# jonnylaw/bayesian_dlms

Measured on AMD Instinct MI355X. Metric: Kalman filter+smooth series*timesteps/sec, higher is better.
Workload: dtype f64

## Files before the change

### bayesian_dlms_amd/csrc/dlm_engine.hip

```cpp
#include "../../include/dlm_engine.h"
#include <cstdlib>
#include "dlm_internal.h"
#include "dlm_draws.h"

#include <rccl/rccl.h>

#include <cstdio>
#include <cstring>
#include <map>
#include <mutex>
#include <set>
#include <string>
#include <vector>

using dlm::KArgs;

namespace dlm {
namespace {
struct LdsEntry {
  size_t granted = 0;
  long long whole = -1;
};
std::mutex lds_mutex;
std::map<std::pair<const void*, int>, LdsEntry> lds_book;
size_t limit_locked(int dev) {
  LdsEntry& lim = lds_book[{nullptr, dev}];
  if (!lim.granted) {
    int v = 0;
    if (hipDeviceGetAttribute(&v, hipDeviceAttributeMaxSharedMemoryPerBlock, dev) != hipSuccess) { (void)hipGetLastError(); v = 0; }
    lim.granted = v > 0 ? (size_t)v : 0;
  }
  return lim.granted;
}
hipError_t opt_in_locked(const void* fn, int dev, size_t bytes) {
  if (bytes > limit_locked(dev)) return hipErrorInvalidValue;
  LdsEntry& en = lds_book[{fn, dev}];
  if (bytes <= en.granted) return hipSuccess;
  const hipError_t err = hipFuncSetAttribute(fn, hipFuncAttributeMaxDynamicSharedMemorySize, (int)bytes);
  if (err == hipSuccess) en.granted = bytes;
  return err;
}
}
size_t lds_limit() {
  int dev = 0;
  if (hipGetDevice(&dev) != hipSuccess) { (void)hipGetLastError(); return 0; }
  std::lock_guard<std::mutex> lock(lds_mutex);
  return limit_locked(dev);
}
hipError_t lds_opt_in(const void* fn, size_t bytes) {
  int dev = 0;
  const hipError_t err = hipGetDevice(&dev);
  if (err != hipSuccess) return err;
  std::lock_guard<std::mutex> lock(lds_mutex);
  return opt_in_locked(fn, dev, bytes);
}
size_t whole_cu_lds(const void* fn) {
  int dev = 0;
  if (hipGetDevice(&dev) != hipSuccess) { (void)hipGetLastError(); return 0; }
  std::lock_guard<std::mutex> lock(lds_mutex);
  LdsEntry& en = lds_book[{fn, dev}];
  if (en.whole < 0) {
    en.whole = 0;
    hipFuncAttributes at;
    const size_t whole = limit_locked(dev);
    if (hipFuncGetAttributes(&at, fn) != hipSuccess) (void)hipGetLastError();
    else if (at.sharedSizeBytes < whole) {
      if (opt_in_locked(fn, dev, whole - at.sharedSizeBytes) == hipSuccess) en.whole = (long long)(whole - at.sharedSizeBytes);
      else (void)hipGetLastError();
    }
  }
  return (size_t)en.whole;
}
}

struct Workspace {
  void* p = nullptr;
  size_t bytes = 0;
  Workspace* next;
  explicit Workspace(Workspace*& list) : next(list) { list = this; }
};
template <class T>
struct Ws : Workspace {
  using Workspace::Workspace;
  operator T*() const { return (T*)p; }
};

struct dlm_engine {
  int device = 0;
  hipStream_t own_stream = nullptr;
  hipStream_t stream = nullptr;
  std::string err;
  const char* variant = "none";
  hipEvent_t ev[3] = {nullptr, nullptr, nullptr};
  bool timed = false;
  Workspace* workspaces = nullptr;
  Ws<void> arena{workspaces};
  Ws<dlm::SparseT> sp_dev{workspaces};
  Ws<dlm::SparseBig> spb_dev{workspaces};
  Ws<double> fws{workspaces}, side{workspaces}, xplus{workspaces}, ystar{workspaces}, covws{workspaces};
  Ws<unsigned char> route{workspaces}, plainbuf{workspaces};
  Ws<void> sampws{workspaces};
  Ws<double> zws{workspaces};
  Ws<void> rtsws{workspaces};
  dlm::SparseF* spf_dev = nullptr;
  int sparse_k = 0;
  ncclComm_t comm = nullptr;
  bool has_comm = false;
  std::set<void*> buffers;
  hipEvent_t order_ev = nullptr;
  struct Analysis {
    bool valid = false;
    int d = 0, p = 0, n_g = 0, branch = 0;
    long long f_stride = 0;
    unsigned generic = 0;
    int sparse_k = 0, spb_k = 0, spf_k = 0;
    bool have_spb = false, have_spf = false;
    std::vector<double> g_host, f_host;
  } an;
  bool an_touched = true;
  bool rts_last = false;
  hipStream_t rng_stream = nullptr;
  hipEvent_t rng_ev = nullptr;
  hipStream_t cov_stream = nullptr;
  hipEvent_t cov_ev[2] = {nullptr, nullptr};
// ... 324 lines not shown
  HIP_TRY(e, hipMemcpyAsync(e->sp_dev, tabs.data(), tabs.size() * sizeof(dlm::SparseT), hipMemcpyHostToDevice, e->stream));
  HIP_TRY(e, hipStreamSynchronize(e->stream));
  e->sparse_k = K;
  return DLM_OK;
}

int mark(dlm_engine* e, int i) {
  HIP_TRY(e, hipEventRecord(e->ev[i], e->stream));
  if (i == 2) e->timed = true;
  return DLM_OK;
}

int ensure_side(dlm_engine* e, size_t N, size_t T) { return ensure(e, e->side, sizeof(double) * 3 * N * (T + 1)); }

int ensure_xplus(dlm_engine* e, const KArgs& k) { return ensure(e, e->xplus, sizeof(double) * (size_t)k.N * ((size_t)k.T + 1) * (size_t)k.d); }

int ensure_ystar(dlm_engine* e, const KArgs& k) {
  return ensure(e, e->ystar, sizeof(double) * (size_t)k.N * (size_t)k.T * (size_t)k.p + (((size_t)k.N * (size_t)(k.T + 1) + 15) & ~(size_t)15));
}

int packed_path(dlm_engine* e, KArgs& k) {
  k.flags |= DLM_OPT_NO_LANE;
  if (!(fast_shape_ok(k) && e->sparse_k > 0) || (k.flags & DLM_OPT_SMOOTHER_COMPAT_Q1))
    return fail(e, DLM_ERR_UNSUPPORTED, "DLM_OPT_PACKED_SYM needs the structured d <= 15, p = 1 path (time-invariant F, <= 4 nonzeros per row and column of G) without DLM_OPT_FORCE_GENERIC / DLM_OPT_SMOOTHER_COMPAT_Q1; use dense records otherwise");
  return DLM_OK;
}

bool use_shared_cov(const dlm_engine* e, const KArgs& k) {
  return fast_shape_ok(k) && e->sparse_k > 0 && !dlm::lane_supported(k) && dlm::shared_cov_eligible(k);
}
size_t route_pad(size_t N) { return (N + 63) & ~(size_t)63; }
int ensure_route(dlm_engine* e, size_t N) { return ensure(e, e->route, route_pad(N) + N * sizeof(int)); }
int* leave_of(dlm_engine* e, size_t N) { return (int*)(e->route + route_pad(N)); }
int mark_plain(dlm_engine* e, KArgs& k) {
  k.plain = nullptr;
  if (!(fast_shape_ok(k) && e->sparse_k > 0) || use_lane(k) || !k.y || k.g_index || k.dt || k.f_stride || k.v_tstride || k.w_tstride ||
      (k.flags & DLM_OPT_NO_STEADY)) return DLM_OK;
  { const int rc = ensure(e, e->plainbuf, (size_t)k.N); if (rc) return rc; }
  HIP_TRY(e, dlm::launch_sparse16_count_gaps(k, e->plainbuf, e->stream));
  k.plain = e->plainbuf;
  return DLM_OK;
}
int ensure_cov_stream(dlm_engine* e) {
  if (!e->cov_stream) {
    int lo = 0, hi = 0;
    HIP_TRY(e, hipDeviceGetStreamPriorityRange(&lo, &hi));
    HIP_TRY(e, hipStreamCreateWithPriority(&e->cov_stream, hipStreamNonBlocking, hi));
    for (auto& ev : e->cov_ev) HIP_TRY(e, hipEventCreateWithFlags(&ev, hipEventDisableTiming));
    HIP_TRY(e, hipEventCreateWithFlags(&e->cov_ev2, hipEventDisableTiming));
    HIP_TRY(e, hipEventCreateWithFlags(&e->rts_ev, hipEventDisableTiming));
  }
  return DLM_OK;
}
int start_sampler_normals(dlm_engine* e, const KArgs& k, dlm::SampTabs& tb, bool big, hipEvent_t gate);
int start_sampler_tables(dlm_engine* e, const KArgs& k, dlm::SampTabs& tb, bool big, const double* crec = nullptr, int crec_stride = 0, bool defer_normals = false) {
  int rc = ensure(e, e->sampws, big ? dlm::wave48_sampler_shared_ws_bytes(k) : dlm::sampler_shared_ws_bytes(k));
  if (rc || (rc = ensure_route(e, (size_t)k.N)) || (rc = ensure_cov_stream(e))) return rc;
  if (big) dlm::wave48_sampler_shared_carve(e->sampws, k, tb); else dlm::sampler_shared_carve(e->sampws, k, tb);
  if ((rc = aux_fork(e, e->cov_stream, e->cov_busy, e->cov_ev[0]))) return rc;
  tb.zstride = 0; tb.mc4 = nullptr; tb.marked = 0;
  if (big) HIP_TRY(e, dlm::launch_wave48_sampler_shared_tables(k, tb, e->cov_stream, e->cov_ev2));
  else if (crec) HIP_TRY(e, dlm::launch_sampler_shared_tables_from(k, e->sparse_k, e->sp_dev, tb, crec, crec_stride, e->cov_stream));
  else HIP_TRY(e, dlm::launch_sampler_shared_tables(k, e->sparse_k, e->sp_dev, tb, e->cov_stream));
  tb.z4 = nullptr;
  if (defer_normals) return DLM_OK;
  return start_sampler_normals(e, k, tb, big, e->cov_ev[0]);
}
int start_sampler_normals(dlm_engine* e, const KArgs& k, dlm::SampTabs& tb, bool big, hipEvent_t gate) {
  if (!k.z) {
    int rc = ensure(e, e->zws, big ? dlm::wave48_sampler_shared_normals_bytes(k) : dlm::sampler_shared_normals_bytes(k));
    if (rc) return rc;
    if (!e->rng_stream) {
      HIP_TRY(e, hipStreamCreateWithFlags(&e->rng_stream, hipStreamNonBlocking));
      HIP_TRY(e, hipEventCreateWithFlags(&e->rng_ev, hipEventDisableTiming));
    }
    if ((rc = aux_fork(e, e->rng_stream, e->rng_busy, gate, false))) return rc;
    if (big) HIP_TRY(e, dlm::launch_wave48_sampler_shared_normals(k, e->zws, e->rng_stream));
    else HIP_TRY(e, dlm::launch_sampler_shared_normals(k, e->zws, e->rng_stream));
    tb.z4 = e->zws;
  }
  return DLM_OK;
}
int start_rts_tables(dlm_engine* e, const KArgs& k, dlm::RtsTabs& tb) {
  bool fresh = false;
  int rc = ensure(e, e->rtsws, dlm::rts_shared_ws_bytes(k), &fresh);
  if (rc) return rc;
  if (fresh) HIP_TRY(e, hipMemsetAsync(e->rtsws, 0, 64, e->stream));
  if ((rc = ensure(e, e->covws, sizeof(double) * dlm::covtabs_doubles(k.d, k.T)))) return rc;
  if ((rc = ensure_route(e, (size_t)k.N)) || (rc = ensure_cov_stream(e))) return rc;
  dlm::RtsKeep keep{};
  dlm::rts_shared_carve(e->rtsws, k, tb, keep);
  dlm::CovTabs ctb{};
  dlm::covtabs_carve(e->covws, k.d, k.T, ctb);
  const bool no_reuse = (k.flags & DLM_OPT_NO_TABLE_REUSE) != 0;
  const int* gate = keep.ctl + dlm::RTS_CTL_GATE;
  e->rts_last = true;
  HIP_TRY(e, dlm::launch_rts_shared_mark(k, e->route, tb, e->stream));
  HIP_TRY(e, dlm::launch_rts_key_check(k, e->sparse_k, e->sp_dev, keep, no_reuse, e->stream));
  HIP_TRY(e, dlm::launch_rts_shared_cov(k, e->sparse_k, e->sp_dev, tb, ctb, gate, e->stream));
  if ((rc = aux_fork(e, e->cov_stream, e->cov_busy, e->cov_ev[0]))) return rc;
  HIP_TRY(e, dlm::launch_rts_shared_tables(k, e->sparse_k, e->sp_dev, tb, gate, e->cov_stream));
  HIP_TRY(e, dlm::launch_rts_key_commit(k, e->sparse_k, e->sp_dev, keep, no_reuse, e->cov_stream));
  HIP_TRY(e, hipEventRecord(e->rts_ev, e->cov_stream));
  HIP_TRY(e, dlm::launch_rts_broadcast(k, e->route, tb, e->cov_stream));
  return DLM_OK;
}
int ensure_shared(dlm_engine* e, const KArgs& k, dlm::CovTabs& tb, bool with_backward) {
  int rc = ensure(e, e->covws, sizeof(double) * dlm::covtabs_doubles(k.d, k.T));
  if (rc || (rc = ensure_route(e, (size_t)k.N)) || (rc = ensure_side(e, k.N, k.T)) || (rc = ensure_cov_stream(e))) return rc;
  dlm::covtabs_carve(e->covws, k.d, k.T, tb);
  tb.eq = e->side + 2 * (size_t)k.N * ((size_t)k.T + 1);
  tb.mc = tb.sc = nullptr;
  if (with_backward) {
    const size_t one = 64 * (size_t)((k.N + 3) / 4) * ((size_t)k.T + 1);
    if ((rc = ensure(e, e->xplus, sizeof(double) * one))) return rc;
    tb.mc = e->xplus;
  }
  return DLM_OK;
}
int run_shared_filter(dlm_engine* e, KArgs& k, dlm::CovTabs& tb, bool with_backward) {
  int rc = ensure_shared(e, k, tb, with_backward);
  if (rc) return rc;
  k.route = e->route; k.route_take = 0;
  e->variant = "sparse16";
  HIP_TRY(e, dlm::launch_sparse16_cov_filter(k, e->sparse_k, e->sp_dev, tb, e->stream));
  if (with_backward) {
    if ((rc = aux_fork(e, e->cov_stream, e->cov_busy, e->cov_ev[0]))) return rc;
    HIP_TRY(e, dlm::launch_sparse16_cov_smoother(k, e->sparse_k, e->sp_dev, tb, e->cov_stream));
  }
  HIP_TRY(e, dlm::launch_sparse16_mean_filter(k, e->sparse_k, e->sp_dev, tb, e->stream));
  KArgs kg = k;
  kg.route_take = 1;
  HIP_TRY(e, dlm::launch_sparse16_filter(kg, e->sparse_k, e->sp_dev, with_backward ? e->side : nullptr, nullptr, e->stream));
  return DLM_OK;
}
int run_shared_smoother(dlm_engine* e, KArgs& k, const dlm::CovTabs& tb) {
  { const int rc = join_cov(e); if (rc) return rc; }
  HIP_TRY(e, dlm::launch_sparse16_mean_smoother(k, e->sparse_k, e->sp_dev, tb, e->stream));
  KArgs kg = k;
  kg.route_take = 1;
  HIP_TRY(e, dlm::launch_sparse16_smoother(kg, e->sparse_k, e->sp_dev, e->side, e->stream));
  return DLM_OK;
}

int run_filter(dlm_engine* e, const KArgs& k, bool want_side) {
  if (use_lane(k)) {
    e->variant = "lane";
    HIP_TRY(e, dlm::launch_lane_filter(k, e->stream));
  } else if (use_fast(e, k) && (!k.prior || e->sparse_k)) {
    if (want_side) { int rc = ensure_side(e, k.N, k.T); if (rc) return rc; }
    double* side = want_side ? e->side : nullptr;
    if (e->sparse_k) {
      e->variant = "sparse16";
      HIP_TRY(e, dlm::launch_sparse16_filter(k, e->sparse_k, e->sp_dev, side, nullptr, e->stream));
    } else {
      e->variant = "mfma16";
      HIP_TRY(e, dlm::launch_mfma16_filter(k, side, e->stream));
// ... 954 lines not shown
  if ((rc = mark(e, 2))) return rc;
  return st.finish(opts->flags & DLM_OPT_ASYNC);
}

int dlm_filter_smooth_batch(dlm_engine* e, const dlm_model_desc* model,
                            const dlm_params_desc* params, const double* y,
                            const dlm_options* opts, double* filt, double* smooth,
                            int32_t* status) {
  int rc = check_common(e, model, params, opts);
  if (rc) return rc;
  if (!y || !smooth) return fail(e, DLM_ERR_ARG, "y and smooth are required");
  e->rts_last = false;
  AuxScope aux(e);
  const size_t d = model->d, p = model->p, T = model->T, N = model->N, rec = d + d * d;
  KArgs k{};
  Stager st(e, opts->mem == DLM_MEM_HOST);
  stage_model(st, k, model, params, opts);
  const bool want_packed = (opts->flags & DLM_OPT_PACKED_SYM) != 0;
  const size_t orec = want_packed ? (size_t)dlm_packed_record_doubles((int)d) : rec;
  st.in(&k.y, y, N * T * p);
  st.out(&k.filt, filt, filt ? N * (T + 1) * orec : 0);
  st.out(&k.smooth, smooth, N * (T + 1) * orec);
  st.zeroed_out(&k.status, (int*)status, N);
  if ((rc = st.commit())) return rc;
  if ((rc = analyse_g(e, k, model->G, opts->mem == DLM_MEM_HOST))) return rc;
  if (want_packed && (rc = packed_path(e, k))) return rc;
  bool fused_fast = fast_smoother_ok(e, k) || use_tiled(k);
  if (want_packed) k.packed = 3;
  const bool q1 = (k.flags & DLM_OPT_SMOOTHER_COMPAT_Q1) != 0;
  const bool rts_shared = fast_shape_ok(k) && e->sparse_k > 0 && !use_lane(k) && !k.packed && !(k.flags & DLM_OPT_SHARED_COV) &&
                          (q1 ? !fused_fast : fast_smoother_ok(e, k)) && dlm::rts_shared_eligible(k, !q1) &&
                          ((uintptr_t)k.smooth & 15) == 0;
  if (!filt) {
    k.packed |= (fast_smoother_ok(e, k) && e->sparse_k > 0 && !use_lane(k) && !rts_shared) ? 1 : 0;
    if ((rc = ensure(e, e->fws, (k.packed & 1) ? N * (T + 1) * (size_t)dlm::packed_rec_bytes((int)d) : N * (T + 1) * rec * sizeof(double)))) return rc;
    k.filt = e->fws;
  }
  if ((rc = mark(e, 0))) return rc;
  dlm::RtsTabs rtb{};
  if (rts_shared && (rc = start_rts_tables(e, k, rtb))) return rc;
  if (rts_shared && (k.flags & DLM_OPT_TEST_FAIL_AFTER_TABLES))
    return fail(e, DLM_ERR_UNSUPPORTED, "DLM_OPT_TEST_FAIL_AFTER_TABLES");
  if ((rc = mark_plain(e, k))) return rc;
  if (filt && fast_smoother_ok(e, k) && use_shared_cov(e, k)) {
    dlm::CovTabs tb;
    if ((rc = run_shared_filter(e, k, tb, true))) return rc;
    if ((rc = mark(e, 1))) return rc;
    k.filt_in = k.filt;
    if ((rc = run_shared_smoother(e, k, tb))) return rc;
    if ((rc = mark(e, 2))) return rc;
    return st.finish(opts->flags & DLM_OPT_ASYNC);
  }
  if ((rc = run_filter(e, k, fused_fast))) return rc;
  if (rts_shared) HIP_TRY(e, hipStreamWaitEvent(e->stream, e->rts_ev, 0));
  if ((rc = mark(e, 1))) return rc;
  k.filt_in = k.filt;
  if (rts_shared) {
    k.route = e->route; k.route_take = 0;
    e->variant = "sparse16-rts-shared";
    HIP_TRY(e, dlm::launch_rts_shared_means(k, e->sparse_k, e->sp_dev, rtb, q1, e->stream));
    if (!q1) {
      KArgs kg = k;
      kg.route_take = 1;
      HIP_TRY(e, dlm::launch_sparse16_smoother(kg, e->sparse_k, e->sp_dev, e->side, e->stream));
    }
  } else if ((rc = run_smoother(e, k, fused_fast))) return rc;
  if (rts_shared && (rc = join_cov(e))) return rc;
  if ((rc = mark(e, 2))) return rc;
  return st.finish(opts->flags & DLM_OPT_ASYNC);
}

static int simsmooth_lane(dlm_engine* e, KArgs& k) {
  int rc = ensure_xplus(e, k);
  if (rc) return rc;
  e->variant = "lane-simsmooth";
  HIP_TRY(e, dlm::launch_lane_simsmooth(k, e->xplus, e->stream));
  return (rc = mark(e, 1)) ? rc : mark(e, 2);
}
static int simsmooth_sparse16(dlm_engine* e, KArgs& k) {
  int rc;
  if ((rc = ensure_side(e, k.N, k.T)) || (rc = ensure_xplus(e, k))) return rc;
  e->variant = "sparse16-simsmooth";
  HIP_TRY(e, dlm::launch_sparse16_filter(k, e->sparse_k, e->sp_dev, e->side, e->xplus, e->stream));
  if ((rc = mark(e, 1))) return rc;
  k.filt_in = k.filt;
  HIP_TRY(e, dlm::launch_sparse16_simsmooth(k, e->sparse_k, e->sp_dev, e->side, e->xplus, e->stream));
  return mark(e, 2);
}
static int simsmooth_tiled(dlm_engine* e, KArgs& k) {
  int rc;
  if (k.w_tstride) {
    k.flags |= DLM_OPT_FORCE_WAVE;
    if (!dlm::wave48_simsmooth_supported(k))
      return fail(e, DLM_ERR_UNSUPPORTED, "a W_t stream with DLM_OPT_FFBS_SIMSMOOTH needs a structured G (at most four nonzeros per row and column); the reference-form sampler takes any model");
  }
  if ((rc = ensure_xplus(e, k)) || (rc = ensure_ystar(e, k))) return rc;
  e->variant = dlm::wave48_simsmooth_supported(k) ? "wave-simsmooth" : "tiled-simsmooth";
  HIP_TRY(e, dlm::launch_tiled_simsmooth(k, e->xplus, e->ystar, e->stream));
  return (rc = mark(e, 1)) ? rc : mark(e, 2);
}
static int forward_shared_means(dlm_engine* e, KArgs& k, dlm::SampTabs& stb) {
  int rc;
  dlm::CovTabs ctb;
  if ((rc = ensure_shared(e, k, ctb, true))) return rc;
  k.route = e->route; k.route_take = 0; k.filt = nullptr;
  HIP_TRY(e, dlm::launch_sparse16_cov_filter(k, e->sparse_k, e->sp_dev, ctb, e->stream));
  if ((rc = start_sampler_tables(e, k, stb, false, ctb.ftab, ctb.frow))) return rc;
  if (k.flags & DLM_OPT_TEST_FAIL_AFTER_TABLES) return fail(e, DLM_ERR_UNSUPPORTED, "DLM_OPT_TEST_FAIL_AFTER_TABLES");
  HIP_TRY(e, dlm::launch_sparse16_mean_filter(k, e->sparse_k, e->sp_dev, ctb, e->stream));
  stb.mc4 = ctb.mc;
  KArgs kg = k;
  kg.route_take = 1; kg.filt = e->fws;
  HIP_TRY(e, dlm::launch_sparse16_filter(kg, e->sparse_k, e->sp_dev, nullptr, nullptr, e->stream));
  k.filt_in = e->fws;
  return DLM_OK;
}
static int forward_records(dlm_engine* e, KArgs& k, dlm::SampTabs& stb, bool shared_factors, bool shared_big, bool norec_big) {
  int rc;
  if ((shared_factors || shared_big) && (rc = start_sampler_tables(e, k, stb, shared_big, nullptr, 0, norec_big))) return rc;
  if ((shared_factors || shared_big) && (k.flags & DLM_OPT_TEST_FAIL_AFTER_TABLES))
// ... 244 lines not shown
```

### bayesian_dlms_amd/csrc/dlm_internal.h

```cpp
#pragma once
#include <hip/hip_runtime.h>
#include <stdint.h>
#include <type_traits>
#include "../../include/dlm_engine.h"

namespace dlm {

struct KArgs {
  int d, p, T, N;
  const double* F; long long f_stride;
  const double* G; int n_g; const int* g_index; const double* dt;
  const double* V; long long v_stride;
  const double* W; long long w_stride;
  long long v_tstride, w_tstride;
  const double* m0; long long m0_stride;
  const double* C0; long long c0_stride;
  const double* y;
  const double* z;
  const double* filt_in;
  double* filt;
  double* prior;
  double* fq;
  double* smooth;
  double* theta;
// ... 114 lines not shown
  double* zrec;
  double* zeros;
  unsigned char* need;
  int* status;
  double* z4;
  int zstride;
  const double* mc4;
  int marked;
  double* ktab;
  int* settle;
};
bool sampler_shared_model_ok(const KArgs& a);
bool sampler_shared_eligible(const KArgs& a);
size_t sampler_shared_ws_bytes(const KArgs& a);
void sampler_shared_carve(void* ws, const KArgs& a, SampTabs& tb);
hipError_t launch_sampler_shared_tables(const KArgs& a, int K, const SparseT* tabs_dev, const SampTabs& tb, hipStream_t s);
hipError_t launch_sampler_shared_tables_from(const KArgs& a, int K, const SparseT* tabs_dev, SampTabs tb, const double* crec, int stride, hipStream_t s);
size_t sampler_shared_normals_bytes(const KArgs& a);
hipError_t launch_sampler_shared_normals(const KArgs& a, double* z4, hipStream_t s);
hipError_t launch_sampler_shared_draw(const KArgs& a, int K, const SparseT* tabs_dev, const SampTabs& tb, hipStream_t s);

struct RtsTabs {
  double* jrows;
  double* srec;
  unsigned char* need;
  int* status;
  const double* crec;
  int crec_stride;
  int* gaps;
  int* skip;
};
constexpr unsigned RTS_KEY_FLAGS = (1u << 0) | (1u << 22);
struct RtsKeySrc {
  int d, T, K;
  unsigned flags;
  const double *F, *V, *W, *C0;
  const SparseT* sp;
};
enum { RTS_CTL_HIT = 10,
       RTS_CTL_GATE = 11,
       RTS_CTL_VALID = 12,
       RTS_CTL_LAST = 13 };
struct RtsKeep { int* ctl; unsigned* key; };
constexpr int RTS_KEY_WORDS = 8 + 2 * (15 + 1 + 2 * 15 * 15) + 2 * (int)(sizeof(SparseT) / 4);
bool rts_shared_eligible(const KArgs& a, bool textbook);
size_t rts_shared_ws_bytes(const KArgs& a);
void rts_shared_carve(void* ws, const KArgs& a, RtsTabs& tb, RtsKeep& keep);
hipError_t launch_rts_key_check(const KArgs& a, int K, const SparseT* tabs_dev, const RtsKeep& keep, bool no_reuse, hipStream_t s);
hipError_t launch_rts_key_commit(const KArgs& a, int K, const SparseT* tabs_dev, const RtsKeep& keep, bool no_reuse, hipStream_t s);
hipError_t launch_rts_shared_cov(const KArgs& a, int K, const SparseT* tabs_dev, RtsTabs& tb, const CovTabs& ctb, const int* gate, hipStream_t s);
hipError_t launch_rts_shared_tables(const KArgs& a, int K, const SparseT* tabs_dev, const RtsTabs& tb, const int* gate, hipStream_t s);
hipError_t launch_rts_shared_mark(const KArgs& a, unsigned char* route, const RtsTabs& tb, hipStream_t s);
hipError_t launch_rts_shared_means(const KArgs& a, int K, const SparseT* tabs_dev, const RtsTabs& tb, bool own_rts, hipStream_t s);
hipError_t launch_rts_broadcast(const KArgs& a, const unsigned char* route, const RtsTabs& tb, hipStream_t s);

bool wave48_sampler_shared_model_ok(const KArgs& a);
bool wave48_sampler_shared_eligible(const KArgs& a);
size_t wave48_sampler_shared_ws_bytes(const KArgs& a);
void wave48_sampler_shared_carve(void* ws, const KArgs& a, SampTabs& tb);
hipError_t launch_wave48_sampler_shared_tables(const KArgs& a, const SampTabs& tb, hipStream_t s, hipEvent_t after_filter = nullptr);
hipError_t launch_wave48_sampler_shared_draw(const KArgs& a, const SampTabs& tb, hipStream_t s);
size_t wave48_ktab_doubles(const KArgs& a);
hipError_t launch_wave48_steady_filter(const KArgs& a, const double* ktab, const int* settle, hipStream_t s);
hipError_t launch_wave48_mark_gaps(const KArgs& a, unsigned char* route, hipStream_t s);
size_t wave48_sampler_shared_normals_bytes(const KArgs& a);
hipError_t launch_wave48_sampler_shared_normals(const KArgs& a, double* z, hipStream_t s);

struct SparseBig { int K; int pad; int idx[48][4]; double val[48][4]; };
int sparse48_analyse(const double* G_host, int d, SparseBig* rows, SparseBig* cols);
struct SparseF { int K; int pad; int cidx[32][4]; double cval[32][4]; int ridx[48][4]; double rval[48][4]; };
int sparsef_analyse(const double* F_host, int d, int p, SparseF* out);
bool tiled_supported(const KArgs& a);
hipError_t launch_tiled_filter(const KArgs& a, double* innov, hipStream_t s);
hipError_t launch_tiled_smoother(const KArgs& a, const double* innov, hipStream_t s);
bool wave48_small_shape(const KArgs& a);
bool wave48_small_ok(const KArgs& a);
bool wave48_filter_supported(const KArgs& a);
hipError_t launch_wave48_filter(const KArgs& a, int K, double* innov, hipStream_t s);
bool wave48_smoother_supported(const KArgs& a);
hipError_t launch_wave48_smoother(const KArgs& a, int K, const double* innov, hipStream_t s);
bool wave48_simsmooth_supported(const KArgs& a);
hipError_t launch_wave48_simsmooth(const KArgs& a, int K, double* xplus, double* ystar, hipStream_t s);
bool wave48_sampler_supported(const KArgs& a);
hipError_t launch_wave48_sampler(const KArgs& a, hipStream_t s);
hipError_t launch_tiled_simsmooth(const KArgs& a, double* xplus, double* ystar, hipStream_t s);

bool svd_supported(const KArgs& a);
size_t svd_filter_lds_bytes(int d, int p);
hipError_t launch_svd_filter(const KArgs& a, double* svd_rec, hipStream_t s);
hipError_t launch_svd_sampler(const KArgs& a, const double* svd_rec, hipStream_t s);
bool svd_shared_eligible(const KArgs& a);
size_t svd_shared_ws_doubles(const KArgs& a);
hipError_t launch_svd_filter_shared(const KArgs& a, double* svd_rec, double* ws, unsigned char* route, hipStream_t s);

bool lane_supported(const KArgs& a);
hipError_t launch_lane_filter(const KArgs& a, hipStream_t s);
hipError_t launch_lane_smoother(const KArgs& a, hipStream_t s);
hipError_t launch_lane_sampler(const KArgs& a, hipStream_t s);
hipError_t launch_lane_simsmooth(const KArgs& a, double* xplus, hipStream_t s);

hipError_t launch_ar1_ffbs(int N, int T, const double* times, const double* y, const double* v, long long v_stride,
                           const double* sv, long long sv_stride, const double* z, unsigned long long seed,
                           unsigned long long series_offset, double* filt, double* theta, int* status, hipStream_t s);

struct DrawStream { unsigned long long seed, series_offset, iteration; };

hipError_t launch_dinvgamma_step(int d, int p, int N, const double* stats, double av, double bv, double aw, double bw,
// ... 255 lines not shown
```

### bayesian_dlms_amd/csrc/dlm_sampler16.hip

```cpp
#include "dlm_internal.h"
#include "dlm_wave.h"
#include "../../include/dlm_engine.h"

namespace dlm {
namespace s16 {

constexpr int IL = 17;
constexpr int IMG = 16 * IL;

__device__ __forceinline__ d4 mm(const d4& x, const d4& y, int rows) {
  d4 acc = {0.0, 0.0, 0.0, 0.0};
#pragma unroll
  for (int r = 0; r < 4; ++r)
    if (4 * r < rows) acc = __builtin_amdgcn_mfma_f64_16x16x4f64(x[r], y[r], acc, 0, 0, 0);
  return acc;
}
__device__ __forceinline__ void to_img(const d4& x, double* img, int g, int c) {
#pragma unroll
  for (int r = 0; r < 4; ++r) img[(4 * r + g) * IL + c] = x[r];
}
__device__ __forceinline__ d4 transposed(const d4& x, double* img, int g, int c) {
  to_img(x, img, g, c);
  wave_sync();
  d4 y;
// ... 982 lines not shown
  if (nd1) lds_dma<NRJ>(rjt, jring_lds + ((T - 1) & 1) * (RJ_ROW * 8), (T - 1) * (RJ_ROW * 8), lane, nj16);
  double sc;
  {
    vm_wait<0>();
    wave_sync();
    const unsigned sslot = sring_lds + (T & 1) * RT_SLOT, mslot = mring_lds + (T & (SF_AHEAD - 1)) * 512;
    double mr = lds_read64<0>(mslot + lane * 8), td = lds_read64<0>(sslot + ptd);
    asm volatile("s_waitcnt lgkmcnt(0)" : "+v"(mr), "+v"(td)::"memory");
    sc = vc ? mr : 0.0;
    vH[lane] = vc ? mr : td;
    wave_sync();
    emit(T, sslot, jring_lds + (T & 1) * (RJ_ROW * 8), mslot, nd2);
  }
  for (int t = T - 1; t >= 0; --t) {
    nd0 = nd1; nd1 = nd2; nd2 = need_of(t - 2);
    if (nd1) vm_wait<4 + NRJ>(); else vm_wait<4>();
    const unsigned sslot = sring_lds + (t & 1) * RT_SLOT, jslot = jring_lds + (t & 1) * (RJ_ROW * 8), mslot = mring_lds + (t & (SF_AHEAD - 1)) * 512;
    double mr = lds_read64<0>(mslot + lane * 8), td = lds_read64<0>(sslot + ptd);
    double mg[K];
#pragma unroll
    for (int s = 0; s < K; ++s) mg[s] = lds_read64<0>(mslot + idx[s]);
    if constexpr (K == 1) asm volatile("s_waitcnt lgkmcnt(0)" : "+v"(mr), "+v"(td), "+v"(mg[0])::"memory");
    else if constexpr (K == 2) asm volatile("s_waitcnt lgkmcnt(0)" : "+v"(mr), "+v"(td), "+v"(mg[0]), "+v"(mg[1])::"memory");
    else if constexpr (K == 3) asm volatile("s_waitcnt lgkmcnt(0)" : "+v"(mr), "+v"(td), "+v"(mg[0]), "+v"(mg[1]), "+v"(mg[2])::"memory");
    else asm volatile("s_waitcnt lgkmcnt(0)" : "+v"(mr), "+v"(td), "+v"(mg[0]), "+v"(mg[1]), "+v"(mg[2]), "+v"(mg[3])::"memory");
    if (nd0) read_J(jslot);
    const double mc = vc ? mr : 0.0;
    double a1 = 0.0;
#pragma unroll
    for (int s = 0; s < K; ++s) a1 = fma(vc ? mg[s] : 0.0, val[s], a1);
    vU[lane] = vc ? sc - a1 : 0.0;
    wave_sync();
    double ch[4] = {0.0, 0.0, 0.0, 0.0};
#pragma unroll
    for (int r = 0; r < 4; ++r)
#pragma unroll
      for (int g = 0; g < 4; ++g) ch[g] = fma(Jc[4 * r + g], vU[16 * j + 4 * r + g], ch[g]);
    const double scol = mc + ((ch[0] + ch[1]) + (ch[2] + ch[3]));
    vH[lane] = vc ? scol : td;
    wave_sync();
    emit(t, sslot, jslot, mslot, nd2);
    sc = vc ? scol : 0.0;
  }
  vm_wait<0>();
  const int stz = tb.status[0];
  const unsigned long long badl = __ballot(!dead && vc && !isfinite(sc));
  if (!dead && c == 0) {
    const int sj = stz | (((badl >> (16 * j)) & 0xffffull) ? DLM_ST_NONFINITE : 0);
    if (a.status && sj) atomicOr(&a.status[n], sj);
  }
}

__global__ __launch_bounds__(256) void k_rts_broadcast(const double* __restrict__ srec, double* smooth, const unsigned char* __restrict__ route,
                                                       const int* __restrict__ skip, int N, int T, int d, int nch) {
  const int lane = threadIdx.x & 63, w = __builtin_amdgcn_readfirstlane((int)(blockIdx.x * 4 + (threadIdx.x >> 6)));
  if (w >= (T + 1) * nch || *skip != 0) return;
  const int t = w % (T + 1), ch = w / (T + 1);
  const int per = (N + nch - 1) / nch, nb = ch * per, ne = nb + per < N ? nb + per : N;
  const int recb = (d + d * d) * 8;
  const bool lines = rts_split_lines(recb), last = t == T;
  const size_t sbytes = (size_t)(T + 1) * recb;
  d2 pc[2];
  int po[2];
#pragma unroll
  for (int k = 0; k < 2; ++k) {
    const int o = 128 + 16 * (64 * k + lane);
    po[k] = o < recb ? o : -1;
    pc[k] = d2{0.0, 0.0};
    if (o < recb) pc[k] = *(const d2*)((const char*)srec + (size_t)t * recb + o);
  }
  unsigned long long routed = 0;
  for (int n = nb; n < ne; ++n) {
    const int i = (n - nb) & 63;
    if (i == 0) routed = __ballot(n + lane < ne && route[n + lane] != 0);
    if ((routed >> i) & 1ull) continue;
    const __amdgpu_buffer_rsrc_t r = mk_rsrc((char*)smooth + (size_t)n * sbytes, sbytes);
    const int ph = (int)(((unsigned long long)smooth + (unsigned long long)n * sbytes + (unsigned long long)t * recb) & 127ull);
#pragma unroll
    for (int k = 0; k < 2; ++k) bst128(r, (po[k] >= 0 && !rts_head_piece(po[k], ph, recb, lines, last)) ? po[k] : OOB, t * recb, pc[k]);
  }
}

}

template <class Tab>
static hipError_t launch_sampler_t(const KArgs& a, int K, const Tab* tabs_dev, hipStream_t s) {
  return pick<1, 2, 3, 4>(K, [&](auto k) { return launch(s16::k_sampler_sp16<k(), Tab>, dim3(a.N), dim3(64), 0, s, a, tabs_dev, SampTabs{}); });
}
hipError_t launch_sparse16_sampler(const KArgs& a, int K, const SparseT* tabs_dev, hipStream_t s) { return launch_sampler_t(a, K, tabs_dev, s); }

template <class Tab>
static hipError_t launch_rts_t(const KArgs& a, int K, const Tab* tabs_dev, hipStream_t s) {
  return pick<1, 2, 3, 4>(K, [&](auto k) { return launch(s16::k_smoother_rts16<k(), Tab>, dim3(a.N), dim3(64), 0, s, a, tabs_dev, RtsTabs{}); });
}
#ifndef DLM_SAMPLER_SHARED_MIN
#define DLM_SAMPLER_SHARED_MIN 1
#endif
bool sampler_shared_model_ok(const KArgs& a) {
  const size_t rec = (size_t)a.d + (size_t)a.d * a.d;
  return a.d <= 15 && a.p == 1 && !a.g_index && !a.dt && !a.f_stride && !a.v_tstride && !a.w_tstride && !a.v_stride && !a.w_stride && !a.c0_stride &&
         !a.packed && a.T >= 1 && a.T <= 400000 && 4 * ((size_t)a.T + 1) * rec * 8 < ((size_t)1 << 31);
}
bool sampler_shared_eligible(const KArgs& a) {
  return sampler_shared_model_ok(a) && !a.cond && (!a.stats || a.y) &&
         !(a.flags & (DLM_OPT_STATS_OUTER | DLM_OPT_FORCE_GENERIC | DLM_OPT_NO_SAMPLER16 | DLM_OPT_SAMPLER_PER_SERIES)) &&
         (a.N >= DLM_SAMPLER_SHARED_MIN || (a.flags & DLM_OPT_NO_SMALL_BATCH));
}
static size_t up64(size_t x) { return (x + 63) & ~(size_t)63; }
size_t sampler_shared_ws_bytes(const KArgs& a) {
  const size_t n1 = (size_t)a.T + 1, rec = (size_t)a.d + (size_t)a.d * a.d;
  return up64(n1 * s16::SF_ROW * 8) + up64(n1 * rec * 8) + up64((size_t)(a.T > 16 ? a.T : 16) * 8) + up64(n1) + 64;
}
void sampler_shared_carve(void* ws, const KArgs& a, SampTabs& tb) {
  const size_t n1 = (size_t)a.T + 1, rec = (size_t)a.d + (size_t)a.d * a.d;
  char* p = (char*)ws;
  tb.rows = (double*)p;  p += up64(n1 * s16::SF_ROW * 8);
  tb.zrec = (double*)p;  p += up64(n1 * rec * 8);
  tb.zeros = (double*)p; p += up64((size_t)(a.T > 16 ? a.T : 16) * 8);
  tb.need = (unsigned char*)p; p += up64(n1);
  tb.status = (int*)p; tb.settle = tb.status + 1;
}
static hipError_t launch_sampler_table_run(const KArgs& kp, int K, const SparseT* tabs_dev, const SampTabs& tb, hipStream_t s) {
  const dim3 grid(s16::sf_stretches(kp.T));
  return pick<1, 2, 3, 4>(K, [&](auto k) { return launch(s16::k_sampler_sp16<k(), SparseT, true>, grid, dim3(64), 0, s, kp, tabs_dev, tb); });
}
hipError_t launch_sampler_shared_tables(const KArgs& a, int K, const SparseT* tabs_dev, const SampTabs& tb, hipStream_t s) {
  hipError_t err = hipMemsetAsync(tb.zeros, 0, (size_t)(a.T > 16 ? a.T : 16) * 8, s);
  if (err != hipSuccess) return err;
  if ((err = hipMemsetAsync(tb.status, 0, sizeof(int), s)) != hipSuccess) return err;
  KArgs kf = table_run_args(a);
  kf.y = tb.zeros; kf.m0 = tb.zeros; kf.filt = tb.zrec; kf.status = tb.status;
  if ((err = launch_sparse16_filter(kf, K, tabs_dev, nullptr, nullptr, s)) != hipSuccess) return err;
// ... 74 lines not shown
  const size_t n1 = (size_t)a.T + 1, rec = (size_t)a.d + (size_t)a.d * a.d;
  return 64 + rts_key_bytes() + up64(n1 * s16::RJ_ROW * 8) + up64(n1 * rec * 8) + up64(n1);
}
void rts_shared_carve(void* ws, const KArgs& a, RtsTabs& tb, RtsKeep& keep) {
  const size_t n1 = (size_t)a.T + 1, rec = (size_t)a.d + (size_t)a.d * a.d;
  char* p = (char*)ws;
  keep.ctl = (int*)p; p += 64;
  keep.key = (unsigned*)p; p += rts_key_bytes();
  tb.jrows = (double*)p; p += up64(n1 * s16::RJ_ROW * 8);
  tb.srec = (double*)p;  p += up64(n1 * rec * 8);
  tb.need = (unsigned char*)p;
  tb.status = keep.ctl; tb.gaps = tb.status + 8; tb.skip = tb.status + 9;
  tb.crec = nullptr; tb.crec_stride = 0;
}
static RtsKeySrc rts_key_of(const KArgs& a, int K, const SparseT* tabs_dev) {
  RtsKeySrc s;
  s.d = a.d; s.T = a.T; s.K = K; s.flags = a.flags & RTS_KEY_FLAGS;
  s.F = a.F; s.V = a.V; s.W = a.W; s.C0 = a.C0; s.sp = tabs_dev;
  return s;
}
hipError_t launch_rts_key_check(const KArgs& a, int K, const SparseT* tabs_dev, const RtsKeep& keep, bool no_reuse, hipStream_t s) {
  if (a.d < 1 || a.d > 15) return hipErrorInvalidValue;
  return launch(s16::k_rts_key_check, dim3(1), dim3(256), 0, s, rts_key_of(a, K, tabs_dev), (const unsigned*)keep.key, keep.ctl, no_reuse ? 1 : 0);
}
hipError_t launch_rts_key_commit(const KArgs& a, int K, const SparseT* tabs_dev, const RtsKeep& keep, bool no_reuse, hipStream_t s) {
  if (a.d < 1 || a.d > 15) return hipErrorInvalidValue;
  return launch(s16::k_rts_key_commit, dim3(1), dim3(256), 0, s, rts_key_of(a, K, tabs_dev), keep.key, keep.ctl, no_reuse ? 1 : 0);
}
hipError_t launch_rts_shared_cov(const KArgs& a, int K, const SparseT* tabs_dev, RtsTabs& tb, const CovTabs& ctb, const int* gate, hipStream_t s) {
  tb.crec = ctb.ftab; tb.crec_stride = ctb.frow;
  CovTabs cs = ctb;
  cs.skip = gate;
  return launch_sparse16_cov_filter(a, K, tabs_dev, cs, s);
}
hipError_t launch_rts_shared_tables(const KArgs& a, int K, const SparseT* tabs_dev, const RtsTabs& tb0, const int* gate, hipStream_t s) {
  RtsTabs tb = tb0;
  tb.skip = const_cast<int*>(gate);
  KArgs kp = table_run_args(a);
  kp.smooth = tb.srec; kp.status = tb.status;
  return pick<1, 2, 3, 4>(K, [&](auto k) {
    const auto kernel = s16::k_smoother_rts16<k(), SparseT, true>;
    return launch(kernel, dim3(1), dim3(64), whole_cu_lds((const void*)kernel), s, kp, tabs_dev, tb);
  });
}
template <int K>
static hipError_t launch_mean_rts(const KArgs& a, const SparseT* sp, const RtsTabs& tb, hipStream_t s) {
  const dim3 grid((a.N + 3) / 4), blk(64);
  constexpr int shape[5][3] = {{2, 1, 1}, {4, 1, 2}, {6, 2, 2}, {8, 2, 2}, {8, 2, 3}};
  const int d = a.d;
  return pick<0, 1, 2, 3, 4>(d <= 7 ? 0 : d <= 10 ? 1 : d <= 13 ? 2 : d == 14 ? 3 : 4, [&](auto c) {
    return launch(s16::k_mean_rts16<K, shape[c()][0], shape[c()][1], shape[c()][2]>, grid, blk, 0, s, a, sp, tb);
  });
}
hipError_t launch_rts_broadcast(const KArgs& a, const unsigned char* route, const RtsTabs& tb, hipStream_t s) {
  if (!route || !a.smooth || a.d < 1 || a.d > 15) return hipErrorInvalidValue;
  const long long rows = (long long)a.T + 1;
  long long nch = (2048 + rows - 1) / rows;
  if (nch > a.N) nch = a.N;
  if (nch < 1) nch = 1;
  return launch(s16::k_rts_broadcast, dim3((unsigned)((rows * nch + 3) / 4)), dim3(256), 0, s, (const double*)tb.srec, a.smooth, route, (const int*)tb.skip, a.N, a.T, a.d, (int)nch);
}
hipError_t launch_rts_shared_mark(const KArgs& a, unsigned char* route, const RtsTabs& tb, hipStream_t s) {
  if (!route || !a.y) return hipErrorInvalidValue;
  hipError_t err = hipMemsetAsync(tb.gaps, 0, 2 * sizeof(int), s);
  if (err != hipSuccess) return err;
  if ((err = launch(s16::k_mark_gaps, dim3((a.N + 3) / 4), dim3(256), 0, s, a.y, a.N, a.T, route, tb.gaps)) != hipSuccess) return err;
  return launch(s16::k_rts_decide, dim3((a.N + 255) / 256), dim3(256), 0, s, route, a.N, (const int*)tb.gaps, tb.skip);
}
hipError_t launch_rts_shared_means(const KArgs& a, int K, const SparseT* tabs_dev, const RtsTabs& tb, bool own_rts, hipStream_t s) {
  if (!a.route || !a.y) return hipErrorInvalidValue;
  hipError_t err;
  KArgs km = a;
  km.route_take = 0;
  err = pick<1, 2, 3, 4>(K, [&](auto k) { return launch_mean_rts<k()>(km, tabs_dev, tb, s); });
  if (err != hipSuccess || !own_rts) return err;
  KArgs kg = a;
  kg.route_take = 1;
  return launch_rts_t(kg, K, tabs_dev, s);
}

hipError_t launch_sparse16_rts(const KArgs& a, int K, const SparseT* tabs_dev, hipStream_t s) { return launch_rts_t(a, K, tabs_dev, s); }
hipError_t launch_small_mv_rts(const KArgs& a, hipStream_t s) { return launch_rts_t(a, a.spb_k, a.spb, s); }
hipError_t launch_small_mv_sampler(const KArgs& a, hipStream_t s) { return launch_sampler_t(a, a.spb_k, a.spb, s); }

}
```

### bayesian_dlms_amd/csrc/dlm_wave.h

```cpp
#pragma once
#include "dlm_internal.h"

namespace dlm {

typedef double d4 __attribute__((ext_vector_type(4)));
typedef double d2 __attribute__((ext_vector_type(2)));
typedef unsigned u2 __attribute__((ext_vector_type(2)));
typedef unsigned u4 __attribute__((ext_vector_type(4)));
typedef int i4 __attribute__((ext_vector_type(4)));

__device__ __forceinline__ void wave_sync() {
  __builtin_amdgcn_fence(__ATOMIC_RELEASE, "wavefront");
  __builtin_amdgcn_wave_barrier();
  __builtin_amdgcn_fence(__ATOMIC_ACQUIRE, "wavefront");
}

template <int CTRL>
__device__ __forceinline__ double dpp_mov(double v) {
  int lo = __double2loint(v), hi = __double2hiint(v);
  lo = __builtin_amdgcn_update_dpp(0, lo, CTRL, 0xf, 0xf, true);
  hi = __builtin_amdgcn_update_dpp(0, hi, CTRL, 0xf, 0xf, true);
  return __hiloint2double(hi, lo);
}
template <int N>
// ... 49 lines not shown
  const u2 l = __builtin_amdgcn_permlane16_swap((unsigned)__double2loint(x), (unsigned)__double2loint(y), false, false);
  const u2 h = __builtin_amdgcn_permlane16_swap((unsigned)__double2hiint(x), (unsigned)__double2hiint(y), false, false);
  lo = __hiloint2double((int)h[0], (int)l[0]);
  hi = __hiloint2double((int)h[1], (int)l[1]);
}
__device__ __forceinline__ double readlane_d(double v, int src) {
  const int lo = __builtin_amdgcn_readlane((int)__double2loint(v), src);
  const int hi = __builtin_amdgcn_readlane((int)__double2hiint(v), src);
  return __hiloint2double(hi, lo);
}
__device__ __forceinline__ double row_pick(double v, int lane, int src) {
  const int a_ = ((lane & 48) + src) << 2;
  const int lo = __builtin_amdgcn_ds_bpermute(a_, __double2loint(v)), hi = __builtin_amdgcn_ds_bpermute(a_, __double2hiint(v));
  return __hiloint2double(hi, lo);
}
__device__ __forceinline__ double row_lane0(double v, int lane) {
  const int a = (lane & 48) << 2;
  const int lo = __builtin_amdgcn_ds_bpermute(a, __double2loint(v)), hi = __builtin_amdgcn_ds_bpermute(a, __double2hiint(v));
  return __hiloint2double(hi, lo);
}

__device__ __forceinline__ double fast_rcp(double x) {
  double r = __builtin_amdgcn_rcp(x);
  r = fma(fma(-x, r, 1.0), r, r);
  r = fma(fma(-x, r, 1.0), r, r);
  return r;
}

__device__ __forceinline__ d4 mmT(const d4& x, const d4& y) {
  d4 acc = {0.0, 0.0, 0.0, 0.0};
  acc = __builtin_amdgcn_mfma_f64_16x16x4f64(x[0], y[0], acc, 0, 0, 0);
  acc = __builtin_amdgcn_mfma_f64_16x16x4f64(x[1], y[1], acc, 0, 0, 0);
  acc = __builtin_amdgcn_mfma_f64_16x16x4f64(x[2], y[2], acc, 0, 0, 0);
  acc = __builtin_amdgcn_mfma_f64_16x16x4f64(x[3], y[3], acc, 0, 0, 0);
  return acc;
}

constexpr int OOB = 0x7ffffff0;
__device__ __forceinline__ __amdgpu_buffer_rsrc_t mk_rsrc(const void* p, size_t bytes) {
  return __builtin_amdgcn_make_buffer_rsrc(const_cast<void*>(p), 0, (int)bytes, 0x00020000);
}
__device__ __forceinline__ double bld(__amdgpu_buffer_rsrc_t r, int voff, int soff) {
  const u2 v = __builtin_amdgcn_raw_buffer_load_b64(r, voff, soff, 0);
  return __hiloint2double((int)v[1], (int)v[0]);
}
__device__ __forceinline__ double bld_glc(__amdgpu_buffer_rsrc_t r, int voff, int soff) {
  const u2 v = __builtin_amdgcn_raw_buffer_load_b64(r, voff, soff, 1);
  return __hiloint2double((int)v[1], (int)v[0]);
}
__device__ __forceinline__ void bst(__amdgpu_buffer_rsrc_t r, int voff, int soff, double x) {
  const u2 v = {(unsigned)__double2loint(x), (unsigned)__double2hiint(x)};
  __builtin_amdgcn_raw_buffer_store_b64(v, r, voff, soff, 0);
}
__device__ __forceinline__ d2 bld128(__amdgpu_buffer_rsrc_t r, int voff, int soff) {
  const u4 v = __builtin_amdgcn_raw_buffer_load_b128(r, voff, soff, 0);
  d2 o = {__hiloint2double((int)v[1], (int)v[0]), __hiloint2double((int)v[3], (int)v[2])};
  return o;
}
template <int AUX = 0>
__device__ __forceinline__ void bst128(__amdgpu_buffer_rsrc_t r, int voff, int soff, double x, double y) {
  const u4 v = {(unsigned)__double2loint(x), (unsigned)__double2hiint(x), (unsigned)__double2loint(y), (unsigned)__double2hiint(y)};
  __builtin_amdgcn_raw_buffer_store_b128(v, r, voff, soff, AUX);
}
template <int AUX = 0>
__device__ __forceinline__ void bst128(__amdgpu_buffer_rsrc_t r, int voff, int soff, d2 x) { bst128<AUX>(r, voff, soff, x[0], x[1]); }

__device__ __forceinline__ i4 rsrc_words(const void* p, unsigned bytes) {
  const unsigned long long a = (unsigned long long)p;
  i4 r = {__builtin_amdgcn_readfirstlane((int)(unsigned)a), __builtin_amdgcn_readfirstlane((int)(unsigned)((a >> 32) & 0xffffu)),
          __builtin_amdgcn_readfirstlane((int)bytes), 0x00020000};
  return r;
}
__device__ __forceinline__ unsigned lds_addr_of(const void* p) {
  return (unsigned)(size_t)(__attribute__((address_space(3))) const char*)p;
}
__device__ __forceinline__ void lds_dma_issue(const i4& rs, unsigned lds_addr, int voff, int soff) {
  asm volatile("s_mov_b32 m0, %0\n\ts_nop 0\n\tbuffer_load_dwordx4 %1, %2, %3 offen lds" ::"s"(lds_addr), "v"(voff), "s"(rs), "s"(soff) : "memory");
}
template <int NR>
__device__ __forceinline__ void lds_dma(const i4& rs, unsigned lds_addr, int soff, int lane, int n16) {
  static_assert(NR >= 1 && NR <= 4, "at most 256 pieces");
  const int voff = lane * 16;
  lds_addr = (unsigned)__builtin_amdgcn_readfirstlane((int)lds_addr);
  soff = __builtin_amdgcn_readfirstlane(soff);
  if (lane < n16) asm volatile("s_mov_b32 m0, %0\n\ts_nop 0\n\tbuffer_load_dwordx4 %1, %2, %3 offen lds" ::"s"(lds_addr), "v"(voff), "s"(rs), "s"(soff) : "memory");
  if constexpr (NR > 1) if (lane + 64 < n16) asm volatile("s_mov_b32 m0, %0\n\ts_nop 0\n\tbuffer_load_dwordx4 %1, %2, %3 offen offset:1024 lds" ::"s"(lds_addr), "v"(voff), "s"(rs), "s"(soff) : "memory");
  if constexpr (NR > 2) if (lane + 128 < n16) asm volatile("s_mov_b32 m0, %0\n\ts_nop 0\n\tbuffer_load_dwordx4 %1, %2, %3 offen offset:2048 lds" ::"s"(lds_addr), "v"(voff), "s"(rs), "s"(soff) : "memory");
  if constexpr (NR > 3) if (lane + 192 < n16) asm volatile("s_mov_b32 m0, %0\n\ts_nop 0\n\tbuffer_load_dwordx4 %1, %2, %3 offen offset:3072 lds" ::"s"(lds_addr), "v"(voff), "s"(rs), "s"(soff) : "memory");
}

template <int OFF>
__device__ __forceinline__ double lds_read64(unsigned addr) {
  double v;
  asm volatile("ds_read_b64 %0, %1 offset:%2" : "=v"(v) : "v"(addr), "n"(OFF) : "memory");
  return v;
}
template <int OFF = 0>
__device__ __forceinline__ d2 lds_read128(unsigned addr) {
  d2 v;
  asm volatile("ds_read_b128 %0, %1 offset:%2" : "=v"(v) : "v"(addr), "n"(OFF) : "memory");
  return v;
}
__device__ __forceinline__ void lds_fence(d4& a) { asm volatile("s_waitcnt lgkmcnt(0)" : "+v"(a)::"memory"); }
__device__ __forceinline__ void lds_fence(d4& a, d4& b) { asm volatile("s_waitcnt lgkmcnt(0)" : "+v"(a), "+v"(b)::"memory"); }
__device__ __forceinline__ void lds_wait(d2& a) { asm volatile("s_waitcnt lgkmcnt(0)" : "+v"(a)::"memory"); }
__device__ __forceinline__ void lds_wait(d2& a, d2& b, d2& c) { asm volatile("s_waitcnt lgkmcnt(0)" : "+v"(a), "+v"(b), "+v"(c)::"memory"); }
// ... 30 lines not shown
```

Baseline: 1.771 billion.

## Make RTS broadcast a CU-sized persistent grid with fixed chunks and pacing

Rewrites the RTS table broadcast kernel as a grid-stride loop over fixed 64-series chunks, with the grid capped at a few blocks per CU. When the table key check hits, the kernel runs alongside the forward filter, so it uses fewer waves in that case. Route bytes and table rows are read through buffer loads, and stores are paced with vm_wait. A compile-time option moves the launch onto the rng stream after the filter, but the default keeps it on the cov stream. The aim is to cut bandwidth contention with the concurrent filter and reduce the cost of oversized launches, at the price of less parallelism in the broadcast.

```diff
diff --git a/bayesian_dlms_amd/csrc/dlm_engine.hip b/bayesian_dlms_amd/csrc/dlm_engine.hip
--- a/bayesian_dlms_amd/csrc/dlm_engine.hip
+++ b/bayesian_dlms_amd/csrc/dlm_engine.hip
@@ -70,6 +70,15 @@
     }
   }
   return (size_t)en.whole;
+}
+int device_cu_count() {
+  static std::map<int, int> cu_book;
+  int dev = 0;
+  if (hipGetDevice(&dev) != hipSuccess) { (void)hipGetLastError(); return 0; }
+  std::lock_guard<std::mutex> lock(lds_mutex);
+  int& n = cu_book[dev];
+  if (n <= 0 && hipDeviceGetAttribute(&n, hipDeviceAttributeMultiprocessorCount, dev) != hipSuccess) { (void)hipGetLastError(); n = 0; }
+  return n;
 }
 }
 
@@ -500,6 +509,13 @@
   }
   return DLM_OK;
 }
+int ensure_rng_stream(dlm_engine* e) {
+  if (!e->rng_stream) {
+    HIP_TRY(e, hipStreamCreateWithFlags(&e->rng_stream, hipStreamNonBlocking));
+    HIP_TRY(e, hipEventCreateWithFlags(&e->rng_ev, hipEventDisableTiming));
+  }
+  return DLM_OK;
+}
 int start_sampler_normals(dlm_engine* e, const KArgs& k, dlm::SampTabs& tb, bool big, hipEvent_t gate);
 int start_sampler_tables(dlm_engine* e, const KArgs& k, dlm::SampTabs& tb, bool big, const double* crec = nullptr, int crec_stride = 0, bool defer_normals = false) {
   int rc = ensure(e, e->sampws, big ? dlm::wave48_sampler_shared_ws_bytes(k) : dlm::sampler_shared_ws_bytes(k));
@@ -518,10 +534,7 @@
   if (!k.z) {
     int rc = ensure(e, e->zws, big ? dlm::wave48_sampler_shared_normals_bytes(k) : dlm::sampler_shared_normals_bytes(k));
     if (rc) return rc;
-    if (!e->rng_stream) {
-      HIP_TRY(e, hipStreamCreateWithFlags(&e->rng_stream, hipStreamNonBlocking));
-      HIP_TRY(e, hipEventCreateWithFlags(&e->rng_ev, hipEventDisableTiming));
-    }
+    if ((rc = ensure_rng_stream(e))) return rc;
     if ((rc = aux_fork(e, e->rng_stream, e->rng_busy, gate, false))) return rc;
     if (big) HIP_TRY(e, dlm::launch_wave48_sampler_shared_normals(k, e->zws, e->rng_stream));
     else HIP_TRY(e, dlm::launch_sampler_shared_normals(k, e->zws, e->rng_stream));
@@ -550,7 +563,23 @@
   HIP_TRY(e, dlm::launch_rts_shared_tables(k, e->sparse_k, e->sp_dev, tb, gate, e->cov_stream));
   HIP_TRY(e, dlm::launch_rts_key_commit(k, e->sparse_k, e->sp_dev, keep, no_reuse, e->cov_stream));
   HIP_TRY(e, hipEventRecord(e->rts_ev, e->cov_stream));
-  HIP_TRY(e, dlm::launch_rts_broadcast(k, e->route, tb, e->cov_stream));
+#if DLM_BCAST_COV_STREAM
+  HIP_TRY(e, dlm::launch_rts_broadcast(k, e->route, tb, keep.ctl + dlm::RTS_CTL_HIT, e->cov_stream));
+#else
+  if ((rc = ensure_rng_stream(e))) return rc;
+#endif
+  return DLM_OK;
+}
+int start_rts_broadcast(dlm_engine* e, const KArgs& k, const dlm::RtsTabs& tb) {
+#if !DLM_BCAST_COV_STREAM
+  int rc;
+  if ((rc = aux_fork(e, e->rng_stream, e->rng_busy, e->cov_ev[0], false))) return rc;
+  HIP_TRY(e, hipStreamWaitEvent(e->rng_stream, e->rts_ev, 0));
+  dlm::RtsTabs same{};
+  dlm::RtsKeep keep{};
+  dlm::rts_shared_carve(e->rtsws, k, same, keep);
+  HIP_TRY(e, dlm::launch_rts_broadcast(k, e->route, tb, keep.ctl + dlm::RTS_CTL_HIT, e->rng_stream));
+#endif
   return DLM_OK;
 }
 int ensure_shared(dlm_engine* e, const KArgs& k, dlm::CovTabs& tb, bool with_backward) {
@@ -1611,6 +1640,7 @@
     return st.finish(opts->flags & DLM_OPT_ASYNC);
   }
   if ((rc = run_filter(e, k, fused_fast))) return rc;
+  if (rts_shared && (rc = start_rts_broadcast(e, k, rtb))) return rc;
   if (rts_shared) HIP_TRY(e, hipStreamWaitEvent(e->stream, e->rts_ev, 0));
   if ((rc = mark(e, 1))) return rc;
   k.filt_in = k.filt;
@@ -1624,7 +1654,7 @@
       HIP_TRY(e, dlm::launch_sparse16_smoother(kg, e->sparse_k, e->sp_dev, e->side, e->stream));
     }
   } else if ((rc = run_smoother(e, k, fused_fast))) return rc;
-  if (rts_shared && (rc = join_cov(e))) return rc;
+  if (rts_shared && ((rc = join_cov(e)) || (rc = join_rng(e)))) return rc;
   if ((rc = mark(e, 2))) return rc;
   return st.finish(opts->flags & DLM_OPT_ASYNC);
 }
diff --git a/bayesian_dlms_amd/csrc/dlm_internal.h b/bayesian_dlms_amd/csrc/dlm_internal.h
--- a/bayesian_dlms_amd/csrc/dlm_internal.h
+++ b/bayesian_dlms_amd/csrc/dlm_internal.h
@@ -190,7 +190,36 @@
 hipError_t launch_rts_shared_tables(const KArgs& a, int K, const SparseT* tabs_dev, const RtsTabs& tb, const int* gate, hipStream_t s);
 hipError_t launch_rts_shared_mark(const KArgs& a, unsigned char* route, const RtsTabs& tb, hipStream_t s);
 hipError_t launch_rts_shared_means(const KArgs& a, int K, const SparseT* tabs_dev, const RtsTabs& tb, bool own_rts, hipStream_t s);
-hipError_t launch_rts_broadcast(const KArgs& a, const unsigned char* route, const RtsTabs& tb, hipStream_t s);
+hipError_t launch_rts_broadcast(const KArgs& a, const unsigned char* route, const RtsTabs& tb, const int* hit, hipStream_t s);
+#ifndef DLM_BCAST_BLOCKS_PER_CU
+#define DLM_BCAST_BLOCKS_PER_CU 2
+#endif
+#ifndef DLM_BCAST_BLOCKS_PER_CU_MISS
+#define DLM_BCAST_BLOCKS_PER_CU_MISS 3
+#endif
+#ifndef DLM_BCAST_CHUNK
+#define DLM_BCAST_CHUNK 64
+#endif
+#ifndef DLM_BCAST_LEGACY_GRID
+#define DLM_BCAST_LEGACY_GRID 0
+#endif
+#ifndef DLM_BCAST_PACE_HIT
+#define DLM_BCAST_PACE_HIT 1
+#endif
+#ifndef DLM_BCAST_PACE_MISS
+#define DLM_BCAST_PACE_MISS 1
+#endif
+#ifndef DLM_BCAST_COV_STREAM
+#define DLM_BCAST_COV_STREAM 1
+#endif
+struct RtsItem { int t, n0, n1; };
+__host__ __device__ inline long long rts_bcast_items(int T, int N, int chunk) { return ((long long)T + 1) * (((long long)N + chunk - 1) / chunk); }
+__host__ __device__ inline RtsItem rts_bcast_item(unsigned item, int T, int N, int chunk) {
+  const unsigned rows = (unsigned)T + 1u, ch = item / rows;
+  const unsigned n0 = ch * (unsigned)chunk, n1 = n0 + (unsigned)chunk;
+  return RtsItem{(int)(item - ch * rows), (int)n0, (int)(n1 < (unsigned)N ? n1 : (unsigned)N)};
+}
+int device_cu_count();
 
 bool wave48_sampler_shared_model_ok(const KArgs& a);
 bool wave48_sampler_shared_eligible(const KArgs& a);
diff --git a/bayesian_dlms_amd/csrc/dlm_sampler16.hip b/bayesian_dlms_amd/csrc/dlm_sampler16.hip
--- a/bayesian_dlms_amd/csrc/dlm_sampler16.hip
+++ b/bayesian_dlms_amd/csrc/dlm_sampler16.hip
@@ -1058,32 +1058,52 @@
 }
 
 __global__ __launch_bounds__(256) void k_rts_broadcast(const double* __restrict__ srec, double* smooth, const unsigned char* __restrict__ route,
-                                                       const int* __restrict__ skip, int N, int T, int d, int nch) {
-  const int lane = threadIdx.x & 63, w = __builtin_amdgcn_readfirstlane((int)(blockIdx.x * 4 + (threadIdx.x >> 6)));
-  if (w >= (T + 1) * nch || *skip != 0) return;
-  const int t = w % (T + 1), ch = w / (T + 1);
-  const int per = (N + nch - 1) / nch, nb = ch * per, ne = nb + per < N ? nb + per : N;
+                                                       const int* __restrict__ skip, const int* __restrict__ hit, int N, int T, int d, int chunk, unsigned items, unsigned waves_hit) {
+  const int lane = threadIdx.x & 63;
+  const unsigned w = (unsigned)__builtin_amdgcn_readfirstlane((int)(blockIdx.x * 4 + (threadIdx.x >> 6)));
+  if (w >= items || *skip != 0) return;
+  const bool beside_forward = *hit != 0;
+  const unsigned W = beside_forward && waves_hit < gridDim.x * 4 ? waves_hit : gridDim.x * 4;
+  if (w >= W) return;
   const int recb = (d + d * d) * 8;
-  const bool lines = rts_split_lines(recb), last = t == T;
+  const bool lines = rts_split_lines(recb);
   const size_t sbytes = (size_t)(T + 1) * recb;
-  d2 pc[2];
-  int po[2];
-#pragma unroll
-  for (int k = 0; k < 2; ++k) {
-    const int o = 128 + 16 * (64 * k + lane);
-    po[k] = o < recb ? o : -1;
-    pc[k] = d2{0.0, 0.0};
-    if (o < recb) pc[k] = *(const d2*)((const char*)srec + (size_t)t * recb + o);
-  }
-  unsigned long long routed = 0;
-  for (int n = nb; n < ne; ++n) {
-    const int i = (n - nb) & 63;
-    if (i == 0) routed = __ballot(n + lane < ne && route[n + lane] != 0);
-    if ((routed >> i) & 1ull) continue;
-    const __amdgpu_buffer_rsrc_t r = mk_rsrc((char*)smooth + (size_t)n * sbytes, sbytes);
-    const int ph = (int)(((unsigned long long)smooth + (unsigned long long)n * sbytes + (unsigned long long)t * recb) & 127ull);
-#pragma unroll
-    for (int k = 0; k < 2; ++k) bst128(r, (po[k] >= 0 && !rts_head_piece(po[k], ph, recb, lines, last)) ? po[k] : OOB, t * recb, pc[k]);
+  const int pace = beside_forward ? DLM_BCAST_PACE_HIT : DLM_BCAST_PACE_MISS;
+  const __amdgpu_buffer_rsrc_t rtab = mk_rsrc(srec, sbytes), rroute = mk_rsrc(route, (size_t)N);
+  int oob;
+  asm("s_mov_b32 %0, 0x7ffffff0" : "=s"(oob));
+  static_assert(OOB == 0x7ffffff0, "the literal above");
+  const int o0 = 128 + 16 * lane;
+  auto fresh_o = [&]() { int o = o0; asm volatile("" : "+v"(o)); return o; };
+  for (unsigned item = w; item < items; item += W) {
+    const RtsItem it = rts_bcast_item(item, T, N, chunk);
+    const int t = it.t, nb = it.n0, ne = it.n1;
+    const bool last = t == T;
+    d2 pc[2];
+#pragma unroll
+    for (int k = 0; k < 2; ++k) {
+      const int o = fresh_o() + 1024 * k;
+      pc[k] = bld128(rtab, o < recb ? o : oob, t * recb);
+    }
+    asm volatile("" : "+v"(pc[0]), "+v"(pc[1]));
+    unsigned long long routed = 0;
+    for (int n = nb; n < ne; ++n) {
+      const int i = (n - nb) & 63;
+      if (i == 0) {
+        const int ln = (fresh_o() - 128) >> 4;
+        routed = __ballot(bld8(rroute, n + ln < ne ? ln : oob, n) != 0);
+      }
+      if ((routed >> i) & 1ull) continue;
+      const __amdgpu_buffer_rsrc_t r = mk_rsrc((char*)smooth + (size_t)n * sbytes, sbytes);
+      const int ph = (int)(((unsigned long long)smooth + (unsigned long long)n * sbytes + (unsigned long long)t * recb) & 127ull);
+      if (pace > 0 && i % pace == 0) vm_wait<0>();
+      const int ol = fresh_o();
+#pragma unroll
+      for (int k = 0; k < 2; ++k) {
+        const int o = ol + 1024 * k;
+        bst128(r, (o < recb && !rts_head_piece(o, ph, recb, lines, last)) ? o : oob, t * recb, pc[k]);
+      }
+    }
   }
 }
 
@@ -1264,13 +1284,26 @@
     return launch(s16::k_mean_rts16<K, shape[c()][0], shape[c()][1], shape[c()][2]>, grid, blk, 0, s, a, sp, tb);
   });
 }
-hipError_t launch_rts_broadcast(const KArgs& a, const unsigned char* route, const RtsTabs& tb, hipStream_t s) {
-  if (!route || !a.smooth || a.d < 1 || a.d > 15) return hipErrorInvalidValue;
+hipError_t launch_rts_broadcast(const KArgs& a, const unsigned char* route, const RtsTabs& tb, const int* hit, hipStream_t s) {
+  if (!route || !hit || !a.smooth || a.d < 1 || a.d > 15 || a.N < 1 || a.T < 0) return hipErrorInvalidValue;
+  unsigned waves_hit = 0xffffffffu;
+#if DLM_BCAST_LEGACY_GRID
   const long long rows = (long long)a.T + 1;
-  long long nch = (2048 + rows - 1) / rows;
+  long long nch = DLM_BCAST_LEGACY_GRID == 2 ? 2048 / rows : (2048 + rows - 1) / rows;
   if (nch > a.N) nch = a.N;
   if (nch < 1) nch = 1;
-  return launch(s16::k_rts_broadcast, dim3((unsigned)((rows * nch + 3) / 4)), dim3(256), 0, s, (const double*)tb.srec, a.smooth, route, (const int*)tb.skip, a.N, a.T, a.d, (int)nch);
+  const int chunk = (int)((a.N + nch - 1) / nch);
+  const long long items = rts_bcast_items(a.T, a.N, chunk), blocks = (items + 3) / 4;
+#else
+  const int chunk = DLM_BCAST_CHUNK, cus = device_cu_count();
+  if (cus < 1) return hipErrorInvalidDevice;
+  constexpr int per_cu = DLM_BCAST_BLOCKS_PER_CU_MISS > DLM_BCAST_BLOCKS_PER_CU ? DLM_BCAST_BLOCKS_PER_CU_MISS : DLM_BCAST_BLOCKS_PER_CU;
+  const long long items = rts_bcast_items(a.T, a.N, chunk), all = (long long)per_cu * cus;
+  const long long blocks = (items + 3) / 4 < all ? (items + 3) / 4 : all;
+  waves_hit = 4u * DLM_BCAST_BLOCKS_PER_CU * (unsigned)cus;
+#endif
+  if (items > 0x7fffffffll) return hipErrorInvalidValue;
+  return launch(s16::k_rts_broadcast, dim3((unsigned)blocks), dim3(256), 0, s, (const double*)tb.srec, a.smooth, route, (const int*)tb.skip, hit, a.N, a.T, a.d, chunk, (unsigned)items, waves_hit);
 }
 hipError_t launch_rts_shared_mark(const KArgs& a, unsigned char* route, const RtsTabs& tb, hipStream_t s) {
   if (!route || !a.y) return hipErrorInvalidValue;
diff --git a/bayesian_dlms_amd/csrc/dlm_wave.h b/bayesian_dlms_amd/csrc/dlm_wave.h
--- a/bayesian_dlms_amd/csrc/dlm_wave.h
+++ b/bayesian_dlms_amd/csrc/dlm_wave.h
@@ -125,6 +125,9 @@
   const u2 v = {(unsigned)__double2loint(x), (unsigned)__double2hiint(x)};
   __builtin_amdgcn_raw_buffer_store_b64(v, r, voff, soff, 0);
 }
+__device__ __forceinline__ int bld8(__amdgpu_buffer_rsrc_t r, int voff, int soff) {
+  return (int)__builtin_amdgcn_raw_buffer_load_b8(r, voff, soff, 0);
+}
 __device__ __forceinline__ d2 bld128(__amdgpu_buffer_rsrc_t r, int voff, int soff) {
   const u4 v = __builtin_amdgcn_raw_buffer_load_b128(r, voff, soff, 0);
   d2 o = {__hiloint2double((int)v[1], (int)v[0]), __hiloint2double((int)v[3], (int)v[2])};
```

New measurement: 1.643 billion. -7.2%, worse.
